# CycloneBoy/pdf_table

Measured on AMD Instinct MI355X. Metric: pages/s, higher is better.
Workload: dtype bf16

## Files before the change

pdf_table_amd/csrc/common.h:

```cpp
#pragma once
#include <hip/hip_runtime.h>
#include <stdint.h>
#include <string.h>

#include <map>
#include <string>
#include <vector>

#include "../../include/pdftable_hip.h"
#include "act16.h"

typedef uint16_t bf16_t;

void pt_set_error(const char* fmt, ...);

#define PT_HIP_CHECK(expr)                                                                  \
  do {                                                                                      \
    hipError_t _e = (expr);                                                                 \
    if (_e != hipSuccess) {                                                                 \
      pt_set_error("%s failed: %s (%s:%d)", #expr, hipGetErrorString(_e), __FILE__, __LINE__); \
      return PT_ERR_HIP;                                                                    \
    }                                                                                       \
  } while (0)

// ... 236 lines not shown
bool pt_conv_fuses_hm(const pt_engine* e);
int pt_launch_crnn_conv01(pt_engine* e, const bf16_t* gray, int n, const float* w64x9, const float* b0, const bf16_t* w1, const float* b1, bf16_t* p1,
                          const int* xlimit, const int* xlimit_cols, hipStream_t s);
int pt_launch_dwpw(pt_engine* e, const bf16_t* in, int B, int H, int W, int C, const float* dw_w, const float* dw_b, int k, int stride, int dw_act,
                   const ConvDesc& pw, hipStream_t s);

int pt_launch_stem7x7(pt_engine* e, const bf16_t* in, int B, int H, int W, const bf16_t* w, const float* bias,
                      bf16_t* out, int split, hipStream_t s, int stride = 2, int n_valid = 0);

int pt_launch_det_preprocess(const uint8_t* pages, int n, int h, int w, int nh, int nw, int flavour, int split,
                             bf16_t* out, hipStream_t s);
int pt_launch_dcn_fused(pt_engine* e, const bf16_t* x, const float* om, const bf16_t* w, const float* bias, bf16_t* out,
                        int B, int H, int W, int C, int N, int split, int relu, hipStream_t s, const bf16_t* omw = nullptr, const float* omb = nullptr,
                        const bf16_t* up_in = nullptr, const float* up_w = nullptr, int up_f = 0);
bool pt_dcn_fuses_om(const pt_engine* e, int C, int split);
bool pt_dcn_fuses_up(const pt_engine* e, int C, int N, int split);
int pt_launch_dwconvt_up_add(const bf16_t* in, const float* w, const bf16_t* add, bf16_t* out, int B, int h, int wd, int C, int f, int split,
                             hipStream_t s);
int pt_launch_maxpool3x3s2(const bf16_t* in, int B, int H, int W, int C, bf16_t* out, int split, hipStream_t s);
int pt_launch_stem7x7_pool(pt_engine* e, const bf16_t* in, int B, int H, int W, const bf16_t* w, const float* bias, bf16_t* out,
                           hipStream_t s);
int pt_launch_db_head_final(const bf16_t* in, int B, int H, int W, const void* w4x64, const float* bias, float* prob,
                            float* logits, int split, hipStream_t s);
int pt_launch_db_head_mfma(const bf16_t* in, int B, int H, int W, const bf16_t* w3, const float* b3, const bf16_t* w6,
                           const float* b6, float* prob, float* logits, hipStream_t s, uint32_t* bitmap = nullptr, float thresh = 0.f);
int pt_launch_bitmap(const float* prob, int n, int H, int W, float thresh, int dilate, uint32_t* bitmap,
                     hipStream_t s);
int pt_launch_box_scores(const float* prob, int n, int H, int W, const float* boxes, int nb, float* scores,
                         hipStream_t s);

#define PT_SE_CHUNKS 64
int pt_launch_stem3x3s2(const bf16_t* in, const float* w, const float* b, bf16_t* out, int B, int H, int W, int split,
                        hipStream_t s, int variant);
int pt_launch_dwconv(const bf16_t* in, const float* w, const float* b, bf16_t* out, int B, int H, int W, int C, int k,
                     int stride, int act, int split, hipStream_t s, const float* slope);
int pt_launch_se(const bf16_t* x, const float* w1, const float* b1, const float* w2, const float* b2, float* gate,
                 bf16_t* out, int B, int HW, int C, int split, hipStream_t s, int hidden, int mode, float* part);
int pt_launch_add(const bf16_t* a, const bf16_t* b, bf16_t* out, long long npix, int C, int split, hipStream_t s);
int pt_launch_chan_mean(const bf16_t* x, int B, int HW, int C, int split, float* part, bf16_t* mean, int rows, hipStream_t s);
int pt_pplcnet_forward_net(pt_engine* e, int slot, const bf16_t* x, int n, int H, int W, int textline, float* logits,
                           int* n_classes, hipStream_t s, int arena);
int pt_launch_cls_resize_norm(const uint8_t* base, const pt_cls_image* images, int n, int max_h, int max_w, int OH, int OW,
                              const float* lut, int split, bf16_t* out, hipStream_t s);
int pt_launch_cls_desc_from_lines(const pt_rec_line* lines, const long long* off, int n, pt_cls_image* images, hipStream_t s);
int pt_launch_cls_line_resize_norm(const uint8_t* pages, int ph, int pw, const pt_rec_line* lines, int n, int max_h, int max_w, int OH,
                                   int OW, const float* lut, int split, bf16_t* out, hipStream_t s);
int pt_launch_dbnas_tail(const bf16_t* y, const float* tw, int B, int H4, int W4, int split, float* prob, float* logits,
                         hipStream_t s);
int pt_dbnas_forward_net(pt_engine* e, const bf16_t* x, int n, int H, int W, float* prob, float* logits, hipStream_t s);

int pt_launch_rec_offsets(const pt_rec_line* lines, int n, long long* off, hipStream_t s);
int pt_launch_rec_warp(const uint8_t* pages, int ph, int pw, const pt_rec_line* lines, int n_lines,
                       const long long* pix_off, uint8_t* crops, int max_crop_px, hipStream_t s);
int pt_launch_rec_resize_gray(const uint8_t* crops, const pt_rec_line* lines, const long long* pix_off, int n_lines,
                              int split, bf16_t* out, hipStream_t s);
int pt_launch_rec_pp_resize_norm(const uint8_t* crops, const pt_rec_line* lines, const long long* pix_off,
                                 const pt_rec_pp_item* items, int n_items, int img_h, int max_img_w, const float* lut, float* out,
                                 hipStream_t s);
struct PtCrnnLimits {
  int* lim[6];
  int* cols;
  int* glist;
  int* blist3a;
  int* blist2a;
  int* blist2b;
};
int pt_launch_rows_live_list(const int* lim, int n, int* glist, hipStream_t s);
int pt_launch_crnn_limits(const pt_rec_line* lines, int n, const PtCrnnLimits& L, hipStream_t s);
int pt_launch_crnn_fill(bf16_t* out, const bf16_t* ref, const int* lim, int tile_w, int div, int n, int rows, int W, int cs,
                        hipStream_t s, const int* end_lim = nullptr, int end_tile = 1);
int pt_launch_crnn_conv0_pool(const bf16_t* in, int n, int H, int W, const float* w64x9, const float* bias, int split,
                              bf16_t* out, hipStream_t s, const int* xlim = nullptr);
int pt_launch_maxpool_kxk(const bf16_t* in, int n, int H, int W, int C, int kh, int kw, int h2c, int split, bf16_t* out,
                          hipStream_t s);
int pt_launch_lstm(pt_engine* e, const bf16_t* gx, const bf16_t* whh, bf16_t* hout, int B, int T, int split, hipStream_t s);
int pt_launch_gemm_argmax(const bf16_t* A, long long M, int K, const bf16_t* W, const float* bias, int N, int* ids, float* maxv,
                          hipStream_t s);
int pt_launch_gemm_argmax_x3(const bf16_t* A, long long M, int K, const bf16_t* W3, const float* bias, int N, int n_real, int* ids, float* maxv,
                             void* scratch, hipStream_t s);
int pt_launch_gemm_rows_x3(const bf16_t* A, long long M, int K, const bf16_t* W3, const float* bias, int N, bf16_t* out, int relu, hipStream_t s,
                           const int* tlim = nullptr);
int pt_launch_gemm_rows(const bf16_t* A, long long M, int K, const bf16_t* W, const float* bias, int N, bf16_t* out, int relu,
                        hipStream_t s, const int* tlim = nullptr);
int pt_launch_argmax_reduce(const float* part, long long rows, int ntiles, int* ids, float* maxv, hipStream_t s);
int pt_crnn_forward_net(pt_engine* e, const bf16_t* gray, int n, int32_t* ids, float* maxlogit, hipStream_t s,
                        const pt_rec_line* d_lines = nullptr);

int pt_cvit_forward_net(pt_engine* e, const float* gray, int layout, int n, int32_t* ids, float* maxlogit, hipStream_t s,
                        const int* h_text_w = nullptr);
int pt_launch_rec_resize_gray_f32(const uint8_t* crops, const pt_rec_line* lines, const long long* pix_off, int n_lines, int tw,
                                  float* out, hipStream_t s);

int pt_mtl_backbone_forward_net(pt_engine* e, const bf16_t* x, int n, int H, int W, float* f3, hipStream_t s);
void pt_mtl_release(pt_engine* e);
int pt_mtl_preprocess(pt_engine* e, const uint8_t* pages, int ph, int pw, const pt_tsr_table* tabs, int n, int size, bf16_t* out, hipStream_t s);
int pt_mtl_decoder_config(pt_engine* e, int32_t* out13);
int pt_mtl_structure(pt_engine* e, const float* f3, int n, int hw, float* d_tag_logits, float* d_boxes, int32_t* h_lens, int32_t* h_cell_counts,
                     int force_redecode, hipStream_t s);
int pt_mtl_cells(pt_engine* e, int total, int32_t* d_cell_ids, float* d_cell_prob, float* d_cell_logits, int32_t* h_steps, int force_redecode,
                 hipStream_t s);

int pt_db_forward_net(pt_engine* e, const bf16_t* x, int n, int H, int W, float* prob, float* logits, hipStream_t s, uint32_t* bitmap = nullptr,
                      float thresh = 0.f, int* bitmap_done = nullptr);
int pt_launch_tsr_preprocess(const uint8_t* pages, int ph, int pw, const pt_tsr_table* tabs, int n, int H, int W, int bgr,
                             const float* lut, bf16_t* out, int split, hipStream_t s);
constexpr int PT_TSR_BAND_ALIGN = 64;
int pt_launch_tsr_preprocess_rows(pt_engine* e, const uint8_t* pages, int ph, int pw, const pt_tsr_table* tabs, const int4* runs, int n_runs, int H, int W,
                                  int bgr, const float* lut, bf16_t* out, int split, hipStream_t s);
int pt_launch_tsr_pad_image(const float* lut, int H, int W, bf16_t* out, int split, hipStream_t s);
struct PtBandSrc {
  long long off;
  int row0, k0, k1, pad_;
};
int pt_launch_tsr_band_assemble(pt_engine* e, const PtBandSrc* src, const bf16_t* pad, bf16_t* out, int n, int rows, int row_elems, hipStream_t s);
int pt_lore_plan_bands(const pt_tsr_table* tabs, int n, int inp_h, int inp_w, int max_stack_rows, int margin, pt_tsr_band* out, int* n_stacks,
                       double* row_fraction);
int pt_lore_band_radius();
int pt_lore_norm_lut(pt_engine* e, const float** lut_out);
int pt_lore_warp_forward_decode(pt_engine* e, const uint8_t* pages, int ph, int pw, const pt_tsr_table* h_tabs, const pt_tsr_table* d_tabs, int n, int H,
                                int W, int bgr, int bands, int margin, int wiz_rev, float vis_thresh, int* d_counts, float* d_dets, float* d_logi,
                                bf16_t* l2_out, hipStream_t s);
bool pt_conv_takes_ws64(const pt_engine* e, int B, int Ho, int Wo);
int pt_picodet_forward_net(pt_engine* e, const bf16_t* x, int n, int H, int W, float* h0, float* h1, float* h2, float* h3,
                          hipStream_t s);
int pt_launch_pico_candidates(const float* head, int B, int A, int ncls, int level, float thr_lo, int max_cands, float* cands,
                              int* counts, hipStream_t s);
int pt_lore_decode(pt_engine* e, const float* hm, const float* st, const float* wh, const float* ax, const float* cr,
                   const float* reg, int B, int H, int W, int wiz_rev, float vis_thresh, int* d_counts, float* d_dets,
                   float* d_logi, hipStream_t s);
void pt_lore_mosaic_rows(int B, int* rows_ax, int* rows_cr, int* rows_cell, int* rows_corner);
int pt_lore_decode_peaks(pt_engine* e, const float* hm, int B, int H, int W, int wiz_rev, float vis_thresh, int* d_counts,
                         const int** d_lim_cell, const int** d_lim_corner, hipStream_t s);
int pt_lore_peak_patches(pt_engine* e, const bf16_t* feat, int B, int H, int W, int C, int split, bf16_t* mos_cell,
                         bf16_t* mos_corner, hipStream_t s);
int pt_lore_decode_boxes(pt_engine* e, const float* reg_cell, const float* wh, const float* reg_corner, const float* st, int B,
                         int H, int W, const int** d_lim_ax, const int** d_lim_cr, hipStream_t s);
int pt_lore_patch_gather(pt_engine* e, const bf16_t* feat, int B, int H, int W, int C, int split, bf16_t* mos_ax, bf16_t* mos_cr,
                         hipStream_t s);
int pt_lore_decode_sparse(pt_engine* e, const float* ax_mos, const float* cr_mos, int B, int H, int W, float vis_thresh,
                          int* d_counts, float* d_dets, float* d_logi, hipStream_t s);
int pt_lore_forward_decode(pt_engine* e, const bf16_t* x, int n, int H, int W, int wiz_rev, float vis_thresh, int* d_counts,
                           float* d_dets, float* d_logi, hipStream_t s);
int pt_lore_wireless_forward_net(pt_engine* e, const bf16_t* x, int n, int H, int W, float* hm, float* st, float* wh,
                                 float* ax, float* cr, float* reg, hipStream_t s);
int pt_lore_process(pt_engine* e, const float* d_logi, const float* d_dets, const int32_t* h_counts, int n_tables,
                    int use_2dpe, float* d_logic, float* d_stacked, hipStream_t s);
int pt_lore_forward_net(pt_engine* e, const bf16_t* x, int n, int H, int W, float* hm, float* st, float* wh, float* ax,
                        float* cr, float* reg, hipStream_t s);
__device__ __forceinline__ float pt_heat_sigmoid(float x) { return 1.f / (1.f + expf(-x)); }
int pt_launch_heat_sigmoid(const float* hm, float* sig, long long npix, hipStream_t s);
int pt_lore_decode_sig_map(pt_engine* e, int B, int H, int W, float** d_sig);
constexpr int PT_HEAT_CAP = 16384;
int pt_heat_peaks_topk(const float* hm, int B, int H, int W, float thr0, float thr1, int k0, int k1, float* sig, unsigned long long* keys,
                       int* cnt, unsigned long long* sorted, int* kept, hipStream_t s);
int pt_centernet_net(pt_engine* e, const bf16_t* x, int n, int H, int W, float* hm, float* v2c, float* c2v, float* reg, hipStream_t s);
int pt_docx_net(pt_engine* e, const bf16_t* x, int n, int H, int W, float* cls, float* ftype, float* hm, float* hm_sub, float* reg, float* reg_sub,
                float* wh, float* wh_sub, hipStream_t s);
int pt_centernet_decode_maps(pt_engine* e, const float* hm, const float* v2c, const float* c2v, const float* reg, int B, int H, int W,
                             const double* affine, int* d_counts, float* d_cells, hipStream_t s);

static inline int pt_split(const pt_engine* e) { return e->precision == PT_PRECISION_BF16X3 || e->precision == PT_PRECISION_F16X2; }
static inline int pt_f16x2(const pt_engine* e) { return e->precision == PT_PRECISION_F16X2; }

struct PtProfScope {
  pt_engine* e;
  hipStream_t s;
// ... 33 lines not shown
```

pdf_table_amd/csrc/crnn_model.hip:

```cpp
#include <stdlib.h>

#include "net_ctx.h"

namespace PT_FMT_NS {

namespace {

struct ConvW {
  const PtTensor *w = nullptr, *b = nullptr;
};

int getw(const PtModel& m, const std::string& base, bool x3, ConvW& out) {
  out.w = m.find(base + (x3 ? ".w3" : ".w"));
  out.b = m.find(base + ".b");
  if (!out.w || !out.b) {
    pt_set_error("CRNN weight blob lacks '%s'", base.c_str());
    return PT_ERR_FORMAT;
  }
  return PT_OK;
}

}

namespace {
struct ZeroLine {
  static constexpr size_t GRAY = 0, A0 = GRAY + 32 * 640, P1 = A0 + 16 * 320 * 64, C2A = P1 + 8 * 160 * 128,
                          P2 = C2A + 8 * 160 * 256, C3A = P2 + 4 * 160 * 256, P3 = C3A + 4 * 160 * 512, F = P3 + 160 * 1024,
                          GX = F + 160 * 512, END = GX + 160 * 2048;
};
}

int pt_crnn_forward_net(pt_engine* e, const bf16_t* gray, int n, int32_t* ids, float* maxlogit, hipStream_t s,
                        const pt_rec_line* d_lines) {
  PT_REQUIRE(e && gray && ids && n > 0, "crnn: bad arguments");
  const PtModel* pm = pt_find_model(e, PT_MODEL_CRNN, "CRNN", "PT_MODEL_CRNN");
  if (!pm) return PT_ERR_STATE;
  const PtModel& M = *pm;
  const int x3 = pt_split(e) ? 1 : 0;
  const int m = x3 ? 2 : 1;
  int rc;
  ConvW c1, c2a, c2b, c3a, c3b, c4, xp1, em1, xp2, em2, cls;
#define G(name, dst) if ((rc = getw(M, name, x3 != 0, dst)) != PT_OK) return rc
  G("conv1", c1); G("conv2a", c2a); G("conv2b", c2b); G("conv3a", c3a); G("conv3b", c3b); G("conv4", c4);
  G("lstm1.xproj", xp1); G("lstm1.emb", em1); G("lstm2.xproj", xp2); G("lstm2.emb", em2); G("cls", cls);
#undef G
  const PtTensor* c0w = M.find(x3 ? "conv0.wf32" : "conv0.wbf");
  const PtTensor* c0b = M.find("conv0.b");
  const PtTensor* whh1 = M.find("lstm1.whh");
  const PtTensor* whh2 = M.find("lstm2.whh");
  if (!c0w || !c0b || !whh1 || !whh2) {
    pt_set_error("CRNN weight blob lacks conv0 / lstm tensors");
    return PT_ERR_FORMAT;
  }
  const int T = PT_REC_T, NT = 7680 / 64;

  struct {
    bf16_t *a0, *a1, *p1, *c2a, *c2b, *p2, *c3a, *c3b, *p3, *f, *gx, *h, *e1, *e2;
    float* part;
  } bf;
  rc = pt_arena_plan(e, PT_ARENA_REC, "crnn", [&](auto&& take_bytes) {
    auto take = [&](size_t elems) { return reinterpret_cast<bf16_t*>(take_bytes(elems * m * sizeof(bf16_t))); };
    const size_t N = (size_t)n;
    bf.a0 = take(N * 16 * 320 * 64);
    bf.a1 = take(N * 16 * 320 * 128);
    bf.p1 = take(N * 8 * 160 * 128);
    bf.c2a = take(N * 8 * 160 * 256);
    bf.c2b = take(N * 8 * 160 * 256);
    bf.p2 = take(N * 4 * 160 * 256);
    bf.c3a = take(N * 4 * 160 * 512);
    bf.c3b = take(N * 4 * 160 * 512);
    bf.p3 = take(N * 160 * 1024);
    bf.f = take(N * T * 512);
    bf.gx = take(N * T * 2048);
    bf.h = take(N * T * 512);
    bf.e1 = take(N * T * 256);
    bf.e2 = take(N * T * 512);
    bf.part = reinterpret_cast<float*>(take_bytes(N * T * NT * 2 * sizeof(float)));
  });
  if (rc != PT_OK) return rc;

#define RUN(call) do { if ((rc = (call)) != PT_OK) return rc; } while (0)
  auto conv = [&](const bf16_t* in, int B, int hh, int ww, int cin, const ConvW& cw, int N, int ks, bf16_t* out, int relu) {
    ConvDesc c;
    c.in = in; c.B = B; c.H = hh; c.W = ww; c.Cin = cin; c.w = W(cw.w); c.bias = F(cw.b); c.N = N; c.ks = ks;
    c.stride = 1; c.out = out; c.out_cstride = N * m; c.relu = relu; c.split = x3; c.out_lo_off = N;
    return c;
  };
  static int fused = -1;
  if (fused < 0) {
    const char* ev = getenv("PT_CLS_FUSED");
    fused = ev ? atoi(ev) : 1;
  }
  auto rows_x3 = [&]() {
    const char* ev = getenv("PT_ROWS_X3");
    return x3 && fused && !pt_f16x2(e) && !(ev && ev[0] == '0');
  };
  auto gemm_pipe = [&]() {
    const char* ev = getenv("PT_GEMM_PIPE");
    return !x3 && !(ev && ev[0] == '0');
  };
  auto rows_gemm = [&](const bf16_t* in, int cin, const ConvW& cw, int N, bf16_t* out, int relu, const char* label) -> int {
    if (!x3 && fused && (cin == 256 || (cin == 512 && !gemm_pipe()))) {
      PtProfScope ps(e, s, PT_PROF_CONV1X1, 2.0 * n * T * (double)cin * N, label);
      return pt_launch_gemm_rows(in, (long long)n * T, cin, W(cw.w), F(cw.b), N, out, relu, s);
    }
    if (rows_x3() && (cin == 512 || cin == 256)) {
      char lb[48];
      snprintf(lb, sizeof(lb), "%s x3", label);
      PtProfScope ps(e, s, PT_PROF_CONV1X1, 2.0 * n * T * (double)cin * N, lb);
      return pt_launch_gemm_rows_x3(in, (long long)n * T, cin, W(cw.w), F(cw.b), N, out, relu, s);
    }
    return pt_launch_conv(e, conv(in, 1, n, T, cin, cw, N, 1, out, relu), s);
  };
  int pool_fused = 1;
  {
    const char* ev = getenv("PT_POOL_FUSED");
    if (ev) pool_fused = atoi(ev);
  }
  auto conv_stack = [&](const bf16_t* g, int nn, bf16_t* a0, bf16_t* a1, bf16_t* p1, bf16_t* c2a_o, bf16_t* c2b_o, bf16_t* p2,
                        bf16_t* c3a_o, bf16_t* c3b_o, bf16_t* p3, bf16_t* f_o, bf16_t* gx_o, const PtCrnnLimits* lim,
                        const bf16_t* zl) -> int {
    auto limited = [&](ConvDesc c, int k) {
      if (lim) {
        c.xlimit = lim->lim[k]; c.xlimit_cols = lim->cols + k;
        if (k == 3) c.block_list = lim->blist3a;
        if (k == 4) c.block_list = lim->glist;
        if (k == 1) c.block_list = lim->blist2a;
        if (k == 2) c.block_list = lim->blist2b;
      }
      return c;
    };
    auto fill = [&](bf16_t* out, size_t zoff, int k, int tile_w, int div, int rows, int Wd, int C, int kn, int tn) -> int {
      if (!lim) return PT_OK;
      PtProfScope ps(e, s, PT_PROF_OTHER, 0, "crnn fill");
      return pt_launch_crnn_fill(out, zl + zoff * m, lim->lim[k], tile_w, div, nn, rows, Wd, C * m, s, kn >= 0 ? lim->lim[kn] : nullptr, tn);
    };
    const char* ev01 = getenv("PT_CONV01");
    const bool conv01 = pool_fused && !x3 && !(ev01 && atoi(ev01) == 0);
    if (conv01) {
      RUN(pt_launch_crnn_conv01(e, g, nn, F(c0w), F(c0b), W(c1.w), F(c1.b), p1, lim ? lim->lim[0] : nullptr, lim ? lim->cols + 0 : nullptr, s));
      RUN(fill(p1, ZeroLine::P1, 0, 32, 2, 8, 160, 128, 1, 32));
    } else {
      PtProfScope ps(e, s, PT_PROF_OTHER, 0, "crnn conv0+pool");
      RUN(pt_launch_crnn_conv0_pool(g, nn, PT_REC_H, PT_REC_W, F(c0w), F(c0b), x3, a0, s, lim ? lim->lim[5] : nullptr));
    }
    if (conv01) {
    } else if (pool_fused) {
      ConvDesc c1d = limited(conv(a0, nn, 16, 320, 64, c1, 128, 3, p1, 1), 0);
      c1d.pool = 1;
      RUN(pt_launch_conv(e, c1d, s));
      RUN(fill(p1, ZeroLine::P1, 0, 32, 2, 8, 160, 128, 1, 32));
    } else {
      RUN(pt_launch_conv(e, conv(a0, nn, 16, 320, 64, c1, 128, 3, a1, 1), s));
      RUN(pt_launch_maxpool_kxk(a1, nn, 16, 320, 128, 2, 2, 0, x3, p1, s));
    }
    RUN(pt_launch_conv(e, limited(conv(p1, nn, 8, 160, 128, c2a, 256, 3, c2a_o, 1), 1), s));
    RUN(fill(c2a_o, ZeroLine::C2A, 1, 32, 1, 8, 160, 256, 2, 32));
    if (pool_fused) {
      ConvDesc c2d = limited(conv(c2a_o, nn, 8, 160, 256, c2b, 256, 3, p2, 1), 2);
      c2d.pool = 2;
      RUN(pt_launch_conv(e, c2d, s));
      RUN(fill(p2, ZeroLine::P2, 2, 32, 1, 4, 160, 256, 3, 64));
    } else {
      RUN(pt_launch_conv(e, conv(c2a_o, nn, 8, 160, 256, c2b, 256, 3, c2b_o, 1), s));
      RUN(pt_launch_maxpool_kxk(c2b_o, nn, 8, 160, 256, 2, 1, 0, x3, p2, s));
    }
    RUN(pt_launch_conv(e, limited(conv(p2, nn, 4, 160, 256, c3a, 512, 3, c3a_o, 1), 3), s));
    RUN(fill(c3a_o, ZeroLine::C3A, 3, 32, 1, 4, 160, 512, 4, 64));
    if (pool_fused) {
      ConvDesc c3d = limited(conv(c3a_o, nn, 4, 160, 512, c3b, 512, 3, p3, 1), 4);
      c3d.pool = 3;
      RUN(pt_launch_conv(e, c3d, s));
    } else {
      RUN(pt_launch_conv(e, conv(c3a_o, nn, 4, 160, 512, c3b, 512, 3, c3b_o, 1), s));
      RUN(pt_launch_maxpool_kxk(c3b_o, nn, 4, 160, 512, 2, 1, 1, x3, p3, s));
    }
    {
      ConvDesc c4d = conv(p3, 1, nn, T, 1024, c4, 512, 1, f_o, 1);
      if (lim) { c4d.xlimit_rows = lim->lim[4]; c4d.xlimit_cols = lim->cols + 5; c4d.block_list = lim->glist; }
      RUN(pt_launch_conv(e, c4d, s));
    }
    if ((!x3 && fused && !gemm_pipe()) || rows_x3()) {
      int lim_slot = -1;
      {
        PtProfScope ps(e, s, PT_PROF_CONV1X1, 2.0 * nn * T * 512.0 * 2048, x3 ? "rows gemm 512->2048 x3" : "rows gemm 512->2048");
        if (x3) RUN(pt_launch_gemm_rows_x3(f_o, (long long)nn * T, 512, W(xp1.w), F(xp1.b), 2048, gx_o, 0, s, lim ? lim->glist : nullptr));
        else RUN(pt_launch_gemm_rows(f_o, (long long)nn * T, 512, W(xp1.w), F(xp1.b), 2048, gx_o, 0, s, lim ? lim->glist : nullptr));
        if (lim && ps.idx >= 0 && e->prof.h_lims && e->prof.n_lims < PtProfile::MAX_LIMS) {
          auto& pd = e->prof.pending[ps.idx];
          pd.lim_slot = lim_slot = e->prof.n_lims++;
          pd.rows = nn * T;
        }
      }
      if (lim_slot >= 0) (void)hipMemcpyAsync(e->prof.h_lims + lim_slot, lim->cols + 5, sizeof(int), hipMemcpyDeviceToHost, s);
    } else {
      ConvDesc xd = conv(f_o, 1, nn, T, 512, xp1, 2048, 1, gx_o, 0);
      if (lim) { xd.xlimit_rows = lim->lim[4]; xd.xlimit_cols = lim->cols + 5; xd.block_list = lim->glist; }
      RUN(pt_launch_conv(e, xd, s));
    }
    RUN(fill(gx_o, ZeroLine::GX, 4, 32, 1, 1, 160, 2048, -1, 1));
    return PT_OK;
  };
  const bool ragged = d_lines != nullptr && pool_fused && e->rec_ragged;
  PtCrnnLimits lim;
  const bf16_t* zl = nullptr;
  if (ragged) {
    if (!e->rec_zero_valid[x3]) {
      const size_t bytes = ZeroLine::END * m * sizeof(bf16_t);
      if (!e->rec_zero[x3]) PT_HIP_CHECK(hipMalloc(&e->rec_zero[x3], bytes));
      PT_HIP_CHECK(hipMemsetAsync(e->rec_zero[x3], 0, bytes, s));
      bf16_t* z = reinterpret_cast<bf16_t*>(e->rec_zero[x3]);
      RUN(conv_stack(z + ZeroLine::GRAY * m, 1, z + ZeroLine::A0 * m, nullptr, z + ZeroLine::P1 * m, z + ZeroLine::C2A * m, nullptr,
                     z + ZeroLine::P2 * m, z + ZeroLine::C3A * m, nullptr, z + ZeroLine::P3 * m, z + ZeroLine::F * m,
                     z + ZeroLine::GX * m, nullptr, nullptr));
      e->rec_zero_valid[x3] = true;
      if (!e->rec_zero_ready[x3]) PT_HIP_CHECK(hipEventCreateWithFlags(&e->rec_zero_ready[x3], hipEventDisableTiming));
      PT_HIP_CHECK(hipEventRecord(e->rec_zero_ready[x3], s));
    } else if (e->rec_zero_ready[x3]) {
      PT_HIP_CHECK(hipStreamWaitEvent(s, e->rec_zero_ready[x3], 0));
    }
    zl = reinterpret_cast<const bf16_t*>(e->rec_zero[x3]);
    const size_t need = ((size_t)26 * n + 40) * sizeof(int);
    if (need > e->rec_limits_cap) {
      PT_HIP_CHECK(hipStreamSynchronize(s));
      if (e->rec_limits) PT_HIP_CHECK(hipFree(e->rec_limits));
      e->rec_limits = nullptr;
      PT_HIP_CHECK(hipMalloc(&e->rec_limits, need * 2));
      e->rec_limits_cap = need * 2;
    }
    int* base = reinterpret_cast<int*>(e->rec_limits);
    for (int k = 0; k < 6; ++k) lim.lim[k] = base + (size_t)k * n;
    lim.cols = base + (size_t)6 * n;
    lim.glist = base + (size_t)6 * n + 8;
    lim.blist3a = base + (size_t)11 * n + 16;
    lim.blist2a = base + (size_t)16 * n + 24;
    lim.blist2b = base + (size_t)21 * n + 32;
    {
      PtProfScope ps(e, s, PT_PROF_OTHER, 0, "crnn limits");
      RUN(pt_launch_crnn_limits(d_lines, n, lim, s));
      RUN(pt_launch_rows_live_list(lim.lim[4], n, lim.glist, s));
      RUN(pt_launch_rows_live_list(lim.lim[3], n, lim.blist3a, s));
      RUN(pt_launch_rows_live_list(lim.lim[1], n, lim.blist2a, s));
      RUN(pt_launch_rows_live_list(lim.lim[2], n, lim.blist2b, s));
    }
  }
  RUN(conv_stack(gray, n, bf.a0, bf.a1, bf.p1, bf.c2a, bf.c2b, bf.p2, bf.c3a, bf.c3b, bf.p3, bf.f, bf.gx, ragged ? &lim : nullptr, zl));
  {
    PtProfScope ps(e, s, PT_PROF_OTHER, 0, "lstm1");
    RUN(pt_launch_lstm(e, bf.gx, W(whh1), bf.h, n, T, x3, s));
  }
  RUN(rows_gemm(bf.h, 512, em1, 256, bf.e1, 0, "rows gemm 512->256"));
  RUN(rows_gemm(bf.e1, 256, xp2, 2048, bf.gx, 0, "rows gemm 256->2048"));
  {
    PtProfScope ps(e, s, PT_PROF_OTHER, 0, "lstm2");
    RUN(pt_launch_lstm(e, bf.gx, W(whh2), bf.h, n, T, x3, s));
  }
  RUN(rows_gemm(bf.h, 512, em2, 512, bf.e2, 0, "rows gemm 512->512"));
  const char* cp_ev = getenv("PT_CLS_PIPE");
  const bool cls_pipe = gemm_pipe() && cp_ev && cp_ev[0] == '1';
  if (!x3 && fused && !cls_pipe) {
    PtProfScope ps(e, s, PT_PROF_CONV1X1, 2.0 * n * T * 512.0 * 7680.0, "classifier gemm+argmax");
    RUN(pt_launch_gemm_argmax(bf.e2, (long long)n * T, 512, W(cls.w), F(cls.b), 7680, ids, maxlogit, s));
  } else if (x3 && fused && !pt_f16x2(e) && !(getenv("PT_CLS_X3_REFINE") && atoi(getenv("PT_CLS_X3_REFINE")) == 0)) {
    PtProfScope ps(e, s, PT_PROF_CONV1X1, 2.0 * n * T * 512.0 * 7680.0, "classifier bound+refine x3");
    RUN(pt_launch_gemm_argmax_x3(bf.e2, (long long)n * T, 512, W(cls.w), F(cls.b), 7680, 7680, ids, maxlogit, bf.part, s));
  } else {
    {
      ConvDesc c = conv(bf.e2, 1, n, T, 512, cls, 7680, 1, nullptr, 0);
      c.argmax_part = bf.part;
// ... 11 lines not shown
```

pdf_table_amd/csrc/rec_kernels.hip:

```cpp
#include <math.h>

#include "common.h"

namespace PT_FMT_NS {

typedef __attribute__((ext_vector_type(8))) __bf16 bf16x8;
typedef __attribute__((ext_vector_type(16))) float f32x16;
typedef __attribute__((ext_vector_type(4))) uint32_t u32x4;
typedef __attribute__((ext_vector_type(2))) uint32_t u32x2;

__device__ __forceinline__ float rbf2f(uint32_t bits16) { return a16_to_f32(bits16); }
__device__ __forceinline__ uint32_t rf2bf(float f) { return f32_to_a16(f); }

__global__ __launch_bounds__(256) void rec_warp_kernel(const uint8_t* __restrict__ pages, int ph, int pw,
                                                        const pt_rec_line* __restrict__ lines, int n_lines,
                                                        const long long* __restrict__ pix_off, uint8_t* __restrict__ crops) {
  a16_kernel_enter();
  const int li = blockIdx.y;
  if (li >= n_lines) return;
  const pt_rec_line L = lines[li];
  const int cw = L.crop_w, chh = L.crop_h;
  const long long npx = (long long)cw * chh;
  uint8_t* dst = crops + pix_off[li] * 3;
  const uint8_t* src = pages + (size_t)L.page * ph * pw * 3;
// ... 1514 lines not shown
  int bi = 0;
  for (int t = 0; t < NT; ++t) {
    const int b = t & 1;
    asm volatile("s_waitcnt vmcnt(0)" ::: "memory");
    __syncthreads();
    const bool more = t + 1 < NT;
    const int soff = more ? (int)((long long)(t + 1) * wts * 2) : 0;
    if (tid < 64) sb[(b ^ 1) * 64 + tid] = bias[(more ? t + 1 : t) * 64 + tid];
    const char* wr = smem + b * TILE + lx * P + q * 16;
    f32x16 acc0, acc1;
#pragma unroll
    for (int r = 0; r < 16; ++r) { acc0[r] = 0.f; acc1[r] = 0.f; }
    bf16x8 f0[D + 1], f1[D + 1];
#pragma unroll
    for (int d = 0; d < D; ++d) {
      f0[d] = *reinterpret_cast<const bf16x8*>(wr + d * 32);
      f1[d] = *reinterpret_cast<const bf16x8*>(wr + 32 * P + d * 32);
    }
#pragma unroll
    for (int ks = 0; ks < KSTEPS; ++ks) {
      if (ks + D < KSTEPS) {
        f0[(ks + D) % (D + 1)] = *reinterpret_cast<const bf16x8*>(wr + (ks + D) * 32);
        f1[(ks + D) % (D + 1)] = *reinterpret_cast<const bf16x8*>(wr + 32 * P + (ks + D) * 32);
      }
      acc0 = mfma_32x32x16_a16(f0[ks % (D + 1)], areg[ks], acc0);
      acc1 = mfma_32x32x16_a16(f1[ks % (D + 1)], areg[ks], acc1);
      if ((ks & 3) == 0)
        __builtin_amdgcn_raw_ptr_buffer_load_lds(r_w, (__attribute__((address_space(3))) void*)(smem + (b ^ 1) * TILE + (wave + 8 * (ks >> 2)) * P), 16,
                                                 more ? voff[ks >> 2] : OOB, soff, 0, 0);
    }
    __builtin_amdgcn_sched_group_barrier(0x100, 2 * D, 0);
#pragma unroll
    for (int ks = 0; ks < KSTEPS; ++ks) {
      __builtin_amdgcn_sched_group_barrier(0x008, 1, 0);
      if (ks + D < KSTEPS) __builtin_amdgcn_sched_group_barrier(0x100, 1, 0);
      __builtin_amdgcn_sched_group_barrier(0x008, 1, 0);
      if (ks + D < KSTEPS) __builtin_amdgcn_sched_group_barrier(0x100, 1, 0);
      if ((ks & 3) == 0) __builtin_amdgcn_sched_group_barrier(0x020, 1, 0);
    }
    const float* sbt = sb + b * 64;
#pragma unroll
    for (int half = 0; half < 2; ++half)
#pragma unroll
      for (int r = 0; r < 16; ++r) {
        const int cl = half * 32 + (r & 3) + 8 * (r >> 2) + 4 * q;
        const float v = (half ? acc1[r] : acc0[r]) + sbt[cl];
        if (MODE == 0) {
          if (v > bv) { bv = v; bi = t * 64 + cl; }
        } else if (v >= thr) {
          if (cnt < CAND_SLOTS && row < M) cp[1 + cnt] = t * 64 + cl;
          ++cnt;
        }
      }
  }
  if (MODE == 1) {
    if (row < M) cp[0] = cnt;
    return;
  }
  const float ov = __shfl_xor(bv, 32);
  const int oi = __shfl_xor(bi, 32);
  if (ov > bv || (ov == bv && oi < bi)) { bv = ov; bi = oi; }
  if (q == 0 && row < M) {
    ids[row] = bi;
    if (maxv) maxv[row] = bv;
  }
#endif
}

static bool cls_dma() {
  const char* ev = getenv("PT_CLS_DMA");
  return !(ev && ev[0] == '0');
}
constexpr int CLS_DMA_SMEM = 2 * 64 * (512 * 2 + 16) + 2 * 64 * 4;
static int cls_dma_attr() {
  static bool done = false;
  if (!done) {
    PT_HIP_CHECK(hipFuncSetAttribute(reinterpret_cast<const void*>(&cls_argmax_dma_kernel<0>), hipFuncAttributeMaxDynamicSharedMemorySize, CLS_DMA_SMEM));
    PT_HIP_CHECK(hipFuncSetAttribute(reinterpret_cast<const void*>(&cls_argmax_dma_kernel<1>), hipFuncAttributeMaxDynamicSharedMemorySize, CLS_DMA_SMEM));
    done = true;
  }
  return PT_OK;
}


__global__ __launch_bounds__(256) void wnorm_max_kernel(const bf16_t* __restrict__ W3, int N, int K, unsigned* __restrict__ out) {
  a16_kernel_enter();
  __shared__ float smax[4];
  const int wave = threadIdx.x >> 6, lane = threadIdx.x & 63;
  const int nch = K >> 5;
  float best = 0.f;
  for (int r = wave; r < 64; r += 4) {
    const int n = blockIdx.x * 64 + r;
    if (n >= N) break;
    const bf16_t* wt = W3 + (size_t)blockIdx.x * 3 * nch * 2048 + r * 32;
    float ss = 0.f;
    for (int k = lane; k < K; k += 64) {
      const float v = rbf2f(wt[(size_t)(k >> 5) * 2048 + (k & 31)]) + rbf2f(wt[(size_t)(2 * nch + (k >> 5)) * 2048 + (k & 31)]);
      ss += v * v;
    }
#pragma unroll
    for (int off = 32; off >= 1; off >>= 1) ss += __shfl_xor(ss, off);
    best = fmaxf(best, sqrtf(ss) * 1.0001f);
  }
  if (lane == 0) smax[wave] = best;
  __syncthreads();
  if (threadIdx.x == 0)
    atomicMax(out, __float_as_uint(fmaxf(fmaxf(smax[0], smax[1]), fmaxf(smax[2], smax[3]))));
}

template <int KSTEPS>
__global__ __launch_bounds__(256, 2) void gemm_cand_kernel(const bf16_t* __restrict__ A, long long M, int lda,
                                                           const bf16_t* __restrict__ W, long long wts, const float* __restrict__ bias,
                                                           int N, const float* __restrict__ wmax, const float* __restrict__ rowmax,
                                                           int* __restrict__ cand) {
  a16_kernel_enter();
  constexpr int K = KSTEPS * 16, P = K * 2 + 16;
  constexpr int NPF = 64 * K * 2 / 16 / 256;
  extern __shared__ __attribute__((aligned(16))) char smem[];
  char* sw = smem;
  float* sb = reinterpret_cast<float*>(smem + 64 * P);
  const int tid = threadIdx.x, lane = tid & 63, wave = tid >> 6;
  const int lx = lane & 31, q = lane >> 5;
  const long long row = ((long long)blockIdx.x * 4 + wave) * 32 + lx;
  const long long rc = row < M ? row : M - 1;
  bf16x8 areg[KSTEPS];
#pragma unroll
  for (int ks = 0; ks < KSTEPS; ++ks) areg[ks] = *reinterpret_cast<const bf16x8*>(A + rc * lda + ks * 16 + q * 8);
  float thr;
  {
    float ss = 0.f;
#pragma unroll
    for (int ks = 0; ks < KSTEPS; ++ks)
#pragma unroll
      for (int i = 0; i < 8; ++i) {
        const float v = (float)areg[ks][i];
        ss += v * v;
      }
    ss += __shfl_xor(ss, 32);
    thr = rowmax[rc] - 2.f * (0.00390625f * 1.02f + 6.103515625e-05f) * sqrtf(ss) * 1.0001f * wmax[0];
  }
  int* cp = cand + (rc * 2 + q) * (1 + CAND_SLOTS);
  int cnt = 0;
  u32x4 pf[NPF];
  float pb = 0.f;
  auto prefetch = [&](int t) {
    const bf16_t* wt = W + (size_t)t * wts;
#pragma unroll
    for (int j = 0; j < NPF; ++j) pf[j] = *reinterpret_cast<const u32x4*>(wt + (size_t)(tid + j * 256) * 8);
    if (tid < 64) pb = bias[t * 64 + tid];
  };
  auto commit = [&]() {
#pragma unroll
    for (int j = 0; j < NPF; ++j) {
      const int idx = tid + j * 256, c = idx >> 8, r = (idx & 255) >> 2, part = idx & 3;
      *reinterpret_cast<u32x4*>(sw + r * P + c * 64 + part * 16) = pf[j];
    }
    if (tid < 64) sb[tid] = pb;
  };
  const int NT = N / 64;
  prefetch(0);
  for (int t = 0; t < NT; ++t) {
    __syncthreads();
    commit();
    __syncthreads();
    if (t + 1 < NT) prefetch(t + 1);
#pragma unroll
// ... 156 lines not shown
  if (!attr0) {
    PT_HIP_CHECK(hipFuncSetAttribute(reinterpret_cast<const void*>(&gemm_argmax_kernel<32, 0, 8>), hipFuncAttributeMaxDynamicSharedMemorySize, SMEM));
    attr0 = true;
  }
  PT_HIP_CHECK(hipMemsetAsync(wmax, 0, 8, s));
  hipLaunchKernelGGL(wnorm_max_kernel, dim3(N / 64), dim3(256), 0, s, W3, N, K, wmax);
  const long long wts = (long long)3 * (K / 32) * 2048;
  if (cls_dma()) {
    if (cls_dma_attr() != PT_OK) return PT_ERR_HIP;
    hipLaunchKernelGGL(cls_argmax_dma_kernel<0>, dim3((unsigned)((M + 255) / 256)), dim3(512), CLS_DMA_SMEM, s, A, M, W3, bias, N, ids, rowmax, 2 * K, wts, nullptr, nullptr, nullptr);
  } else {
    hipLaunchKernelGGL((gemm_argmax_kernel<32, 0, 8>), dim3((unsigned)((M + 255) / 256)), dim3(512), SMEM, s, A, M, W3, bias, N, ids, rowmax, nullptr, 0,
                       nullptr, 2 * K, wts);
  }
  if (cls_dma())
    hipLaunchKernelGGL(cls_argmax_dma_kernel<1>, dim3((unsigned)((M + 255) / 256)), dim3(512), CLS_DMA_SMEM, s, A, M, W3, bias, N, nullptr, nullptr, 2 * K, wts,
                       reinterpret_cast<const float*>(wmax), rowmax, cand);
  else
    hipLaunchKernelGGL((gemm_cand_kernel<32>), dim3((unsigned)((M + 127) / 128)), dim3(256), SMEM, s, A, M, 2 * K, W3, wts, bias, N,
                       reinterpret_cast<const float*>(wmax), rowmax, cand);
  hipLaunchKernelGGL(cand_eval_kernel, dim3((unsigned)((M + 15) / 16)), dim3(256), 0, s, A, M, 2 * K, K, W3, bias, N, n_real, cand, ids, maxv, ovf_count,
                     ovf_rows);
  hipLaunchKernelGGL(cand_full_kernel, dim3(2048), dim3(256), 0, s, A, 2 * K, K, W3, bias, n_real, ovf_count, ovf_rows, ids, maxv);
  PT_HIP_CHECK(hipGetLastError());
  return PT_OK;
}

static int gemm_nw(int dflt) {
  static int nw = -1;
  if (nw < 0) {
    const char* ev = getenv("PT_GEMM_NW");
    nw = ev ? (atoi(ev) == 8 ? 8 : 4) : 0;
  }
  return nw ? nw : dflt;
}

int pt_launch_gemm_argmax(const bf16_t* A, long long M, int K, const bf16_t* W, const float* bias, int N, int* ids, float* maxv,
                          hipStream_t s) {
  if ((K != 512 && K != 192) || N % 64 != 0 || M <= 0) return PT_ERR_INVALID;
  constexpr int SMEM = 64 * (512 * 2 + 16) + 64 * 4;
  static bool attr_done = false;
  if (!attr_done) {
    PT_HIP_CHECK(hipFuncSetAttribute(reinterpret_cast<const void*>(&gemm_argmax_kernel<32, 0>), hipFuncAttributeMaxDynamicSharedMemorySize, SMEM));
    PT_HIP_CHECK(hipFuncSetAttribute(reinterpret_cast<const void*>(&gemm_argmax_kernel<12, 0>), hipFuncAttributeMaxDynamicSharedMemorySize, SMEM));
    PT_HIP_CHECK(hipFuncSetAttribute(reinterpret_cast<const void*>(&gemm_argmax_kernel<32, 0, 8>), hipFuncAttributeMaxDynamicSharedMemorySize, SMEM));
    PT_HIP_CHECK(hipFuncSetAttribute(reinterpret_cast<const void*>(&gemm_argmax_kernel<12, 0, 8>), hipFuncAttributeMaxDynamicSharedMemorySize, SMEM));
    attr_done = true;
  }
  const int nw = gemm_nw(K == 512 ? 8 : 4);
  const dim3 grid((unsigned)((M + nw * 32 - 1) / (nw * 32))), blk(nw * 64);
  if (K == 192) {
    if (nw == 8) hipLaunchKernelGGL((gemm_argmax_kernel<12, 0, 8>), grid, blk, 64 * (192 * 2 + 16) + 64 * 4, s, A, M, W, bias, N, ids, maxv, nullptr, 0, nullptr, 192, 6ll * 2048);
    else hipLaunchKernelGGL((gemm_argmax_kernel<12, 0>), grid, blk, 64 * (192 * 2 + 16) + 64 * 4, s, A, M, W, bias, N, ids, maxv, nullptr, 0, nullptr, 192, 6ll * 2048);
  } else {
    if (nw == 8 && cls_dma()) {
      if (cls_dma_attr() != PT_OK) return PT_ERR_HIP;
      hipLaunchKernelGGL(cls_argmax_dma_kernel<0>, grid, blk, CLS_DMA_SMEM, s, A, M, W, bias, N, ids, maxv, 512, 16ll * 2048, nullptr, nullptr, nullptr);
    } else if (nw == 8) hipLaunchKernelGGL((gemm_argmax_kernel<32, 0, 8>), grid, blk, SMEM, s, A, M, W, bias, N, ids, maxv, nullptr, 0, nullptr, 512, 16ll * 2048);
    else hipLaunchKernelGGL((gemm_argmax_kernel<32, 0>), grid, blk, SMEM, s, A, M, W, bias, N, ids, maxv, nullptr, 0, nullptr, 512, 16ll * 2048);
  }
  PT_HIP_CHECK(hipGetLastError());
  return PT_OK;
}

int pt_launch_gemm_rows(const bf16_t* A, long long M, int K, const bf16_t* W, const float* bias, int N, bf16_t* out, int relu,
                        hipStream_t s, const int* tlim) {
  if ((K != 512 && K != 256) || N % 64 != 0 || M <= 0) return PT_ERR_INVALID;
  const int nw = gemm_nw(4);
  const int smem = 64 * (K * 2 + 16) + 64 * 4 + nw * 32 * 80;
  static bool attr_done = false;
  if (!attr_done) {
    PT_HIP_CHECK(hipFuncSetAttribute(reinterpret_cast<const void*>(&gemm_argmax_kernel<32, 1>), hipFuncAttributeMaxDynamicSharedMemorySize, 64 * (512 * 2 + 16) + 256 + 4 * 32 * 80));
    PT_HIP_CHECK(hipFuncSetAttribute(reinterpret_cast<const void*>(&gemm_argmax_kernel<32, 1, 8>), hipFuncAttributeMaxDynamicSharedMemorySize, 64 * (512 * 2 + 16) + 256 + 8 * 32 * 80));
    attr_done = true;
  }
  const dim3 grid((unsigned)((M + nw * 32 - 1) / (nw * 32))), blk(nw * 64);
  if (K == 512) {
    if (nw == 8) hipLaunchKernelGGL((gemm_argmax_kernel<32, 1, 8>), grid, blk, smem, s, A, M, W, bias, N, nullptr, nullptr, out, relu, tlim, 512, 16ll * 2048);
    else hipLaunchKernelGGL((gemm_argmax_kernel<32, 1>), grid, blk, smem, s, A, M, W, bias, N, nullptr, nullptr, out, relu, tlim, 512, 16ll * 2048);
  } else {
    if (nw == 8) hipLaunchKernelGGL((gemm_argmax_kernel<16, 1, 8>), grid, blk, smem, s, A, M, W, bias, N, nullptr, nullptr, out, relu, tlim, 256, 8ll * 2048);
    else hipLaunchKernelGGL((gemm_argmax_kernel<16, 1>), grid, blk, smem, s, A, M, W, bias, N, nullptr, nullptr, out, relu, tlim, 256, 8ll * 2048);
  }
  PT_HIP_CHECK(hipGetLastError());
  return PT_OK;
}

template <int KSTEPS>
__global__ __launch_bounds__(256, KSTEPS == 32 ? 1 : 2) void gemm_rows_x3_kernel(const bf16_t* __restrict__ A, long long M, const bf16_t* __restrict__ W3,
                                                                                 const float* __restrict__ bias, int N, bf16_t* __restrict__ out, int relu,
                                                                                 const int* __restrict__ tlim) {
  a16_kernel_enter();
  constexpr int K = KSTEPS * 16, NCH = K / 32, P = K * 2 + 16;
  constexpr int NPF = NCH;
  extern __shared__ __attribute__((aligned(16))) char smem[];
  char* sw = smem;
  float* sb = reinterpret_cast<float*>(smem + 64 * P);
  const int tid = threadIdx.x, lane = tid & 63, wave = tid >> 6;
  const int lx = lane & 31, q = lane >> 5;
  long long row0 = ((long long)blockIdx.x * 4 + wave) * 32;
  bool live = row0 < M;
  if (tlim) {
    const int total = tlim[0], g = blockIdx.x * 4 + wave;
    if ((int)blockIdx.x * 4 >= total) return;
    live = g < total;
    row0 = live ? (long long)tlim[1 + g] * 32 : 0;
  }
  const long long row = row0 + lx;
  const long long rc = row < M ? row : M - 1;
  bf16x8 ahi[KSTEPS], alo[KSTEPS];
#pragma unroll
  for (int ks = 0; ks < KSTEPS; ++ks) {
    ahi[ks] = *reinterpret_cast<const bf16x8*>(A + rc * (2 * K) + ks * 16 + q * 8);
    alo[ks] = *reinterpret_cast<const bf16x8*>(A + rc * (2 * K) + K + ks * 16 + q * 8);
  }
  u32x4 pf[NPF];
  float pb = 0.f;
  auto prefetch = [&](int st) {
    const bf16_t* wt = W3 + (size_t)(st >> 1) * (3 * NCH * 2048) + (st & 1) * (32 * 32);
#pragma unroll
    for (int j = 0; j < NPF; ++j) {
      const int idx = tid + j * 256, plane = idx / (NCH * 128), rem = idx - plane * (NCH * 128), c = rem >> 7, rp = rem & 127;
      pf[j] = *reinterpret_cast<const u32x4*>(wt + (size_t)(plane * 2 * NCH + c) * 2048 + rp * 8);
    }
    if (tid < 32) pb = bias[st * 32 + tid];
  };
  auto commit = [&]() {
#pragma unroll
    for (int j = 0; j < NPF; ++j) {
      const int idx = tid + j * 256, plane = idx / (NCH * 128), rem = idx - plane * (NCH * 128), c = rem >> 7, r = (rem & 127) >> 2, part = rem & 3;
      *reinterpret_cast<u32x4*>(sw + (plane * 32 + r) * P + c * 64 + part * 16) = pf[j];
    }
    if (tid < 32) sb[tid] = pb;
  };
  char* tile = smem + 64 * P + 128 + wave * (2 * 32 * 80);
  const int NS = N / 32;
  prefetch(0);
  for (int st = 0; st < NS; ++st) {
    __syncthreads();
    commit();
    __syncthreads();
    if (st + 1 < NS) prefetch(st + 1);
    if (!live) continue;
    f32x16 acc;
#pragma unroll
    for (int r = 0; r < 16; ++r) acc[r] = 0.f;
    const char* wh = sw + lx * P + q * 16;
    const char* wl = sw + (32 + lx) * P + q * 16;
#pragma unroll
    for (int ks = 0; ks < KSTEPS; ++ks) {
      acc = mfma_32x32x16_a16(*reinterpret_cast<const bf16x8*>(wh + ks * 32), ahi[ks], acc);
      if ((ks & 7) == 7) __builtin_amdgcn_sched_barrier(0);
    }
#pragma unroll
    for (int ks = 0; ks < KSTEPS; ++ks) {
      acc = mfma_32x32x16_a16(*reinterpret_cast<const bf16x8*>(wh + ks * 32), alo[ks], acc);
      if ((ks & 7) == 7) __builtin_amdgcn_sched_barrier(0);
    }
#pragma unroll
    for (int ks = 0; ks < KSTEPS; ++ks) {
      acc = mfma_32x32x16_a16(*reinterpret_cast<const bf16x8*>(wl + ks * 32), ahi[ks], acc);
      if ((ks & 7) == 7) __builtin_amdgcn_sched_barrier(0);
    }
#pragma unroll
    for (int rg = 0; rg < 4; ++rg) {
      const int cl = rg * 8 + 4 * q;
// ... 56 lines not shown
```

Baseline: 843.5.

## Add double-buffered LDS-DMA rows GEMM kernel for 512-wide CRNN projections

Adds a new rows GEMM kernel that streams weight tiles straight into LDS through buffer_load_lds DMA. The loads are double-buffered, so the next N-tile's weights and bias arrive while MFMAs run on the current tile, with 8 waves per workgroup. The kernel is enabled by default for cin=512 with N=2048 or 512, including the LSTM input projection. It is meant to hide weight-load latency and cut register-staged copies, at the cost of one workgroup per CU, heavy LDS use, and hand-tuned scheduling barriers.

Result: no change. 845.2, median of 3 (+0.2%).

```diff
diff --git a/pdf_table_amd/csrc/common.h b/pdf_table_amd/csrc/common.h
--- a/pdf_table_amd/csrc/common.h
+++ b/pdf_table_amd/csrc/common.h
@@ -342,6 +342,8 @@
                            const int* tlim = nullptr);
 int pt_launch_gemm_rows(const bf16_t* A, long long M, int K, const bf16_t* W, const float* bias, int N, bf16_t* out, int relu,
                         hipStream_t s, const int* tlim = nullptr);
+int pt_launch_gemm_rows_dma(const bf16_t* A, long long M, int K, const bf16_t* W, const float* bias, int N, bf16_t* out, int relu, hipStream_t s,
+                            const int* tlim = nullptr);
 int pt_launch_argmax_reduce(const float* part, long long rows, int ntiles, int* ids, float* maxv, hipStream_t s);
 int pt_crnn_forward_net(pt_engine* e, const bf16_t* gray, int n, int32_t* ids, float* maxlogit, hipStream_t s,
                         const pt_rec_line* d_lines = nullptr);
diff --git a/pdf_table_amd/csrc/crnn_model.hip b/pdf_table_amd/csrc/crnn_model.hip
--- a/pdf_table_amd/csrc/crnn_model.hip
+++ b/pdf_table_amd/csrc/crnn_model.hip
@@ -99,14 +99,28 @@
     const char* ev = getenv("PT_GEMM_PIPE");
     return !x3 && !(ev && ev[0] == '0');
   };
+  auto rows_dma = [&](int cin, int N) {
+    const char* ev = getenv("PT_ROWS_DMA");
+    if (ev && ev[0] == '0') return false;
+    if (ev && ev[0] == '2') return true;
+    return cin == 512 && (N == 2048 || N == 512);
+  };
+  auto rows_bytes = [&](int rows, int cin, int N) { return 2.0 * rows * ((double)cin + N); };
   auto rows_gemm = [&](const bf16_t* in, int cin, const ConvW& cw, int N, bf16_t* out, int relu, const char* label) -> int {
+    if (!x3 && fused && rows_dma(cin, N)) {
+      e->prof.next_bytes = rows_bytes(n * T, cin, N);
+      PtProfScope ps(e, s, PT_PROF_CONV1X1, 2.0 * n * T * (double)cin * N, label);
+      return pt_launch_gemm_rows_dma(in, (long long)n * T, cin, W(cw.w), F(cw.b), N, out, relu, s);
+    }
     if (!x3 && fused && (cin == 256 || (cin == 512 && !gemm_pipe()))) {
+      e->prof.next_bytes = rows_bytes(n * T, cin, N);
       PtProfScope ps(e, s, PT_PROF_CONV1X1, 2.0 * n * T * (double)cin * N, label);
       return pt_launch_gemm_rows(in, (long long)n * T, cin, W(cw.w), F(cw.b), N, out, relu, s);
     }
     if (rows_x3() && (cin == 512 || cin == 256)) {
       char lb[48];
       snprintf(lb, sizeof(lb), "%s x3", label);
+      e->prof.next_bytes = 2.0 * rows_bytes(n * T, cin, N);
       PtProfScope ps(e, s, PT_PROF_CONV1X1, 2.0 * n * T * (double)cin * N, lb);
       return pt_launch_gemm_rows_x3(in, (long long)n * T, cin, W(cw.w), F(cw.b), N, out, relu, s);
     }
@@ -180,11 +194,14 @@
       if (lim) { c4d.xlimit_rows = lim->lim[4]; c4d.xlimit_cols = lim->cols + 5; c4d.block_list = lim->glist; }
       RUN(pt_launch_conv(e, c4d, s));
     }
-    if ((!x3 && fused && !gemm_pipe()) || rows_x3()) {
+    const bool dma = !x3 && fused && rows_dma(512, 2048);
+    if (dma || (!x3 && fused && !gemm_pipe()) || rows_x3()) {
       int lim_slot = -1;
       {
+        e->prof.next_bytes = (x3 ? 2.0 : 1.0) * rows_bytes(nn * T, 512, 2048);
         PtProfScope ps(e, s, PT_PROF_CONV1X1, 2.0 * nn * T * 512.0 * 2048, x3 ? "rows gemm 512->2048 x3" : "rows gemm 512->2048");
         if (x3) RUN(pt_launch_gemm_rows_x3(f_o, (long long)nn * T, 512, W(xp1.w), F(xp1.b), 2048, gx_o, 0, s, lim ? lim->glist : nullptr));
+        else if (dma) RUN(pt_launch_gemm_rows_dma(f_o, (long long)nn * T, 512, W(xp1.w), F(xp1.b), 2048, gx_o, 0, s, lim ? lim->glist : nullptr));
         else RUN(pt_launch_gemm_rows(f_o, (long long)nn * T, 512, W(xp1.w), F(xp1.b), 2048, gx_o, 0, s, lim ? lim->glist : nullptr));
         if (lim && ps.idx >= 0 && e->prof.h_lims && e->prof.n_lims < PtProfile::MAX_LIMS) {
           auto& pd = e->prof.pending[ps.idx];
diff --git a/pdf_table_amd/csrc/rec_kernels.hip b/pdf_table_amd/csrc/rec_kernels.hip
--- a/pdf_table_amd/csrc/rec_kernels.hip
+++ b/pdf_table_amd/csrc/rec_kernels.hip
@@ -1620,6 +1620,131 @@
   return PT_OK;
 }
 
+template <int KSTEPS>
+__global__ __launch_bounds__(512, 1) void rows_dma_kernel(const bf16_t* __restrict__ A, long long M, const bf16_t* __restrict__ W, const float* __restrict__ bias,
+                                                          int N, bf16_t* __restrict__ out, int relu, const int* __restrict__ tlim) {
+#if defined(__HIP_DEVICE_COMPILE__)
+  a16_kernel_enter();
+  constexpr int NW = 8, K = KSTEPS * 16, RPL = 1024 / (K * 2), LINES = 64 / RPL, PL = 1024 + 16, TILE = LINES * PL, D = 2;
+  constexpr int LPW = LINES / NW, REQ = KSTEPS / LPW;
+  constexpr int HOFF = RPL == 2 ? 512 : 32 * PL;
+  static_assert(LINES % NW == 0 && KSTEPS % LPW == 0 && REQ >= 1, "a tile is whole DMA passes of the workgroup, spread over the k-loop");
+  extern __shared__ __attribute__((aligned(16))) char smem[];
+  float* sb = reinterpret_cast<float*>(smem + 2 * TILE);
+  const int tid = threadIdx.x, lane = tid & 63;
+  const int wave = __builtin_amdgcn_readfirstlane(tid >> 6);
+  const int lx = lane & 31, q = lane >> 5;
+  char* tile = smem + 2 * TILE + 512 + wave * (32 * 80);
+  long long row0 = ((long long)blockIdx.x * NW + wave) * 32;
+  bool live = row0 < M;
+  if (tlim) {
+    const int total = tlim[0], g = blockIdx.x * NW + wave;
+    if ((int)blockIdx.x * NW >= total) return;
+    live = g < total;
+    row0 = live ? (long long)tlim[1 + g] * 32 : 0;
+  }
+  const long long row = row0 + lx;
+  const long long rc = row < M ? row : M - 1;
+  bf16x8 areg[KSTEPS];
+#pragma unroll
+  for (int ks = 0; ks < KSTEPS; ++ks) areg[ks] = *reinterpret_cast<const bf16x8*>(A + rc * K + ks * 16 + q * 8);
+  constexpr int OOB = 0x7FFFF000;
+  const __amdgpu_buffer_rsrc_t r_w = __builtin_amdgcn_make_buffer_rsrc(const_cast<bf16_t*>(W), 0, OOB, 0x00020000);
+  int voff[LPW];
+#pragma unroll
+  for (int j = 0; j < LPW; ++j) {
+    const int ln = wave + NW * j;
+    const int wrow = RPL == 2 ? ln + 32 * q : ln, chunk = RPL == 2 ? lx >> 2 : lane >> 2;
+    voff[j] = (((chunk * 64 + wrow) * 32) + (lane & 3) * 8) * 2;
+  }
+  const int NT = N / 64;
+  const long long wts = (long long)(K / 32) * 2048;
+#pragma unroll
+  for (int j = 0; j < LPW; ++j)
+    __builtin_amdgcn_raw_ptr_buffer_load_lds(r_w, (__attribute__((address_space(3))) void*)(smem + (wave + NW * j) * PL), 16, voff[j], 0, 0, 0);
+  const __amdgpu_buffer_rsrc_t r_b = __builtin_amdgcn_make_buffer_rsrc(const_cast<float*>(bias), 0, N * 4, 0x00020000);
+  if (wave == 0) __builtin_amdgcn_raw_ptr_buffer_load_lds(r_b, (__attribute__((address_space(3))) void*)sb, 4, lane * 4, 0, 0, 0);
+  asm volatile("s_waitcnt vmcnt(0) lgkmcnt(0)" ::: "memory");
+  __builtin_amdgcn_s_barrier();
+  asm volatile("" ::: "memory");
+  for (int t = 0; t < NT; ++t) {
+    const int b = t & 1;
+    const bool more = t + 1 < NT;
+    const int soff = more ? (int)((long long)(t + 1) * wts * 2) : 0;
+    if (wave == 0)
+      __builtin_amdgcn_raw_ptr_buffer_load_lds(r_b, (__attribute__((address_space(3))) void*)(sb + (b ^ 1) * 64), 4, lane * 4,
+                                               __builtin_amdgcn_readfirstlane((more ? t + 1 : t) * 256), 0, 0);
+    f32x16 acc0, acc1;
+    if (live) {
+      const char* wr = smem + b * TILE + lx * PL + q * 16;
+#pragma unroll
+      for (int r = 0; r < 16; ++r) { acc0[r] = 0.f; acc1[r] = 0.f; }
+      bf16x8 f0[D + 1], f1[D + 1];
+#pragma unroll
+      for (int d = 0; d < D; ++d) {
+        f0[d] = *reinterpret_cast<const bf16x8*>(wr + d * 32);
+        f1[d] = *reinterpret_cast<const bf16x8*>(wr + HOFF + d * 32);
+      }
+#pragma unroll
+      for (int ks = 0; ks < KSTEPS; ++ks) {
+        if (ks + D < KSTEPS) {
+          f0[(ks + D) % (D + 1)] = *reinterpret_cast<const bf16x8*>(wr + (ks + D) * 32);
+          f1[(ks + D) % (D + 1)] = *reinterpret_cast<const bf16x8*>(wr + HOFF + (ks + D) * 32);
+        }
+        acc0 = mfma_32x32x16_a16(f0[ks % (D + 1)], areg[ks], acc0);
+        acc1 = mfma_32x32x16_a16(f1[ks % (D + 1)], areg[ks], acc1);
+        if (ks % REQ == 0)
+          __builtin_amdgcn_raw_ptr_buffer_load_lds(r_w, (__attribute__((address_space(3))) void*)(smem + (b ^ 1) * TILE + (wave + NW * (ks / REQ)) * PL), 16,
+                                                   more ? voff[ks / REQ] : OOB, soff, 0, 0);
+      }
+      __builtin_amdgcn_sched_group_barrier(0x100, 2 * D, 0);
+#pragma unroll
+      for (int ks = 0; ks < KSTEPS; ++ks) {
+        __builtin_amdgcn_sched_group_barrier(0x008, 1, 0);
+        if (ks + D < KSTEPS) __builtin_amdgcn_sched_group_barrier(0x100, 1, 0);
+        __builtin_amdgcn_sched_group_barrier(0x008, 1, 0);
+        if (ks + D < KSTEPS) __builtin_amdgcn_sched_group_barrier(0x100, 1, 0);
+        if (ks % REQ == 0) __builtin_amdgcn_sched_group_barrier(0x020, 1, 0);
+      }
+    } else {
+#pragma unroll
+      for (int j = 0; j < LPW; ++j)
+        __builtin_amdgcn_raw_ptr_buffer_load_lds(r_w, (__attribute__((address_space(3))) void*)(smem + (b ^ 1) * TILE + (wave + NW * j) * PL), 16,
+                                                 more ? voff[j] : OOB, soff, 0, 0);
+    }
+    asm volatile("s_waitcnt vmcnt(0)" ::: "memory");
+    if (live) {
+      const float* sbt = sb + b * 64;
+#pragma unroll
+      for (int half = 0; half < 2; ++half) {
+#pragma unroll
+        for (int rg = 0; rg < 4; ++rg) {
+          const int cl = half * 32 + rg * 8 + 4 * q;
+          uint32_t hb[4];
+#pragma unroll
+          for (int k = 0; k < 4; ++k) {
+            float v = (half ? acc1[rg * 4 + k] : acc0[rg * 4 + k]) + sbt[cl + k];
+            v = relu ? fmaxf(v, 0.f) : v;
+            hb[k] = rf2bf(v);
+          }
+          *reinterpret_cast<u32x2*>(tile + lx * 80 + (rg * 8 + 4 * q) * 2) = u32x2{hb[0] | (hb[1] << 16), hb[2] | (hb[3] << 16)};
+        }
+        asm volatile("s_waitcnt lgkmcnt(0)" ::: "memory");
+#pragma unroll
+        for (int i = 0; i < 2; ++i) {
+          const int r = (lane >> 2) + 16 * i;
+          const u32x4 v = *reinterpret_cast<const u32x4*>(tile + r * 80 + (lane & 3) * 16);
+          if (row0 + r < M) *reinterpret_cast<u32x4*>(out + (row0 + r) * N + t * 64 + half * 32 + (lane & 3) * 8) = v;
+        }
+        asm volatile("s_waitcnt lgkmcnt(0)" ::: "memory");
+      }
+    }
+    __builtin_amdgcn_s_barrier();
+    asm volatile("" ::: "memory");
+  }
+#endif
+}
+
 
 __global__ __launch_bounds__(256) void wnorm_max_kernel(const bf16_t* __restrict__ W3, int N, int K, unsigned* __restrict__ out) {
   a16_kernel_enter();
@@ -1942,6 +2067,23 @@
     if (nw == 8) hipLaunchKernelGGL((gemm_argmax_kernel<16, 1, 8>), grid, blk, smem, s, A, M, W, bias, N, nullptr, nullptr, out, relu, tlim, 256, 8ll * 2048);
     else hipLaunchKernelGGL((gemm_argmax_kernel<16, 1>), grid, blk, smem, s, A, M, W, bias, N, nullptr, nullptr, out, relu, tlim, 256, 8ll * 2048);
   }
+  PT_HIP_CHECK(hipGetLastError());
+  return PT_OK;
+}
+
+int pt_launch_gemm_rows_dma(const bf16_t* A, long long M, int K, const bf16_t* W, const float* bias, int N, bf16_t* out, int relu, hipStream_t s,
+                            const int* tlim) {
+  if ((K != 512 && K != 256) || N % 64 != 0 || M <= 0 || (relu != 0 && relu != 1)) return PT_ERR_INVALID;
+  const int smem = 2 * (K == 512 ? 64 : 32) * (1024 + 16) + 2 * 64 * 4 + 8 * 32 * 80;
+  static bool attr_done = false;
+  if (!attr_done) {
+    PT_HIP_CHECK(hipFuncSetAttribute(reinterpret_cast<const void*>(&rows_dma_kernel<32>), hipFuncAttributeMaxDynamicSharedMemorySize, 2 * 64 * 1040 + 512 + 8 * 2560));
+    PT_HIP_CHECK(hipFuncSetAttribute(reinterpret_cast<const void*>(&rows_dma_kernel<16>), hipFuncAttributeMaxDynamicSharedMemorySize, 2 * 32 * 1040 + 512 + 8 * 2560));
+    attr_done = true;
+  }
+  const dim3 grid((unsigned)((M + 255) / 256)), blk(512);
+  if (K == 512) hipLaunchKernelGGL((rows_dma_kernel<32>), grid, blk, smem, s, A, M, W, bias, N, out, relu, tlim);
+  else hipLaunchKernelGGL((rows_dma_kernel<16>), grid, blk, smem, s, A, M, W, bias, N, out, relu, tlim);
   PT_HIP_CHECK(hipGetLastError());
   return PT_OK;
 }
```
